# oxfordcontrol/Clarabel.rs

Measured on NVIDIA H100. Metric: ipm_iterations_per_sec, higher is better.
Workload: dtype f64

## Files before the change

clarabel.rs_b200/csrc/ldl.cu:

```cuda
#include <cuda_runtime.h>
#include <dlfcn.h>

#include <cmath>
#include <cstdio>
#include <cstring>
#include <algorithm>
#include <thread>
#include <vector>

#include "../../include/clarabel_b200.h"
#include "ldl_device.h"
#include "symbolic.h"
#include "vec.cuh"

namespace cb {

std::atomic<unsigned long long> g_launches{0};

typedef struct ncclComm* cb_ncclComm_t;
typedef struct { char internal[128]; } cb_ncclUniqueId;
struct NcclApi {
  void* lib = nullptr;
  int (*GetUniqueId)(cb_ncclUniqueId*) = nullptr;
  int (*CommInitRank)(cb_ncclComm_t*, int, cb_ncclUniqueId, int) = nullptr;
  int (*AllGather)(const void*, void*, size_t, int, cb_ncclComm_t, cudaStream_t) = nullptr;
  int (*CommDestroy)(cb_ncclComm_t) = nullptr;
  const char* (*GetErrorString)(int) = nullptr;
};
static NcclApi* nccl_api(const char* libpath) {
  static NcclApi api;
  static bool tried = false;
  if (api.lib) return &api;
  if (tried && !libpath) return nullptr;
  tried = true;
  void* h = dlopen(libpath && *libpath ? libpath : "libnccl.so.2", RTLD_NOW | RTLD_GLOBAL);
  if (!h) { std::fprintf(stderr, "[clarabel_b200] dlopen(%s) failed: %s\n", libpath ? libpath : "libnccl.so.2", dlerror()); return nullptr; }
  api.GetUniqueId = (int (*)(cb_ncclUniqueId*))dlsym(h, "ncclGetUniqueId");
  api.CommInitRank = (int (*)(cb_ncclComm_t*, int, cb_ncclUniqueId, int))dlsym(h, "ncclCommInitRank");
  api.AllGather = (int (*)(const void*, void*, size_t, int, cb_ncclComm_t, cudaStream_t))dlsym(h, "ncclAllGather");
  api.CommDestroy = (int (*)(cb_ncclComm_t))dlsym(h, "ncclCommDestroy");
  api.GetErrorString = (const char* (*)(int))dlsym(h, "ncclGetErrorString");
  if (!api.GetUniqueId || !api.CommInitRank || !api.AllGather || !api.CommDestroy) return nullptr;
  api.lib = h;
  return &api;
}



template <int NT>
__device__ __forceinline__ void pivot_inverse(double* A, int lda, int ns) {
  for (int j = threadIdx.x; j < ns; j += NT) {
    for (int i = j + 1; i < ns; i++) {
      double a0 = A[(long long)j * lda + i], a1 = 0.0;
      int k = j + 1;
      for (; k + 1 < i; k += 2) {
        a0 += A[(long long)k * lda + i] * A[(long long)k * lda + j];
        a1 += A[(long long)(k + 1) * lda + i] * A[(long long)(k + 1) * lda + j];
      }
      if (k < i) a0 += A[(long long)k * lda + i] * A[(long long)k * lda + j];
      A[(long long)i * lda + j] = -(a0 + a1);
    }
  }
}
template <int NT>
__device__ __forceinline__ void pivot_inverse_place(double* A, int lda, int ns) {
  for (int idx = threadIdx.x; idx < ns * ns; idx += NT) {
    const int j = idx / ns, i = idx - j * ns;
    if (i > j) {
      A[(long long)j * lda + i] = A[(long long)i * lda + j];
      A[(long long)i * lda + j] = 0.0;
    }
  }
}

template <int NT>
__global__ void __launch_bounds__(NT) k_factor_level(LDLDev d, int task_base, int smem_cap) {
  extern __shared__ double sm[];
  __shared__ double sD[CB_MAX_PANEL];
  __shared__ double sInv[CB_MAX_PANEL];
  const int tid = threadIdx.x;
  const int lane = tid & 31, warp = tid >> 5, nwarp = NT >> 5;
  const int s = d.level_tasks[task_base + blockIdx.x];
  const int f = d.sn_first[s];
  const int ns = d.sn_first[s + 1] - f;
  const long long rp = d.sn_rowptr[s];
  const int nr = (int)(d.sn_rowptr[s + 1] - rp);
  const int ld = ns + nr;
  double* __restrict__ P = d.L + d.panel_off[s];
  double* __restrict__ U = d.U + d.upd_off[s];
  const long long psz = (long long)ld * ns;
  const bool use_sm = psz <= (long long)smem_cap;
  double* W = use_sm ? sm : P;

  for (long long i = tid; i < psz; i += NT) W[i] = 0.0;
  __syncthreads();
  for (long long e = d.asm_ptr[s] + tid; e < d.asm_ptr[s + 1]; e += NT)
    W[d.asm_dst[e]] = d.vals[d.asm_src[e]];

  int c_reg = 0, c_pos = 0, c_zero = 0, c_nonf = 0;
  for (int j = 0; j < ns; j++) {
    __syncthreads();
    const double* __restrict__ cj = W + (long long)j * ld;
    double dj = cj[j];
    bool reg = false;
    if (d.reg_enable) {
      const double sg = (double)d.dsigns[f + j];
      if (dj * sg < d.reg_eps) { dj = d.reg_delta * sg; reg = true; }
    }
    const double inv = 1.0 / dj;
    if (tid == 0) {
      c_reg += reg ? 1 : 0;
      c_pos += dj > 0.0 ? 1 : 0;
      if (dj == 0.0) c_zero = 1;
      if (!isfinite(inv)) c_nonf = 1;
      d.D[f + j] = dj;
      d.Dinv[f + j] = inv;
      sD[j] = dj;
      sInv[j] = inv;
    }
    for (int k = j + 1 + warp; k < ns; k += nwarp) {
      const double wk = cj[k] * inv;
      double* __restrict__ ck = W + (long long)k * ld;
      for (int i = k + lane; i < ld; i += 32) ck[i] -= cj[i] * wk;
    }
  }
  __syncthreads();
  for (int j = warp; j < ns; j += nwarp) {
    double* __restrict__ cj = W + (long long)j * ld;
    const double inv = sInv[j];
    if (lane == 0) cj[j] = sD[j];
    for (int i = j + 1 + lane; i < ld; i += 32) cj[i] *= inv;
  }
  if (tid == 0) {
    if (c_reg) atomicAdd(&d.status[ST_REGCOUNT], c_reg);
    if (c_pos) atomicAdd(&d.status[ST_POSINERTIA], c_pos);
    if (c_zero) atomicExch(&d.status[ST_ZEROPIV], 1);
    if (c_nonf) atomicExch(&d.status[ST_NONFINITE], 1);
  }
  __syncthreads();

  {
    int it = 0;
    for (int b0 = 0; b0 < nr; b0 += 4)
      for (int a0 = b0; a0 < nr; a0 += 32, it++) {
        if (it % nwarp != warp) continue;
        const int a = a0 + lane;
        const bool on = a < nr;
        const int nb = min(4, nr - b0);
        double acc[4] = {0.0, 0.0, 0.0, 0.0};
        const double* __restrict__ ck = W + ns;
        for (int k = 0; k < ns; k++, ck += ld) {
          const double la = on ? ck[a] : 0.0, dk = sD[k];
#pragma unroll
          for (int c = 0; c < 4; c++) acc[c] += la * (ck[b0 + min(c, nb - 1)] * dk);
        }
#pragma unroll
        for (int c = 0; c < 4; c++)
          if (on && b0 + c < nr && a >= b0 + c) U[(long long)(b0 + c) * nr + a] = 0.0 - acc[c];
      }
  }
  if (ns > CB_SOLVE_SMALL_NS) {
    pivot_inverse<NT>(W, ld, ns);
    __syncthreads();
    pivot_inverse_place<NT>(W, ld, ns);
  }
  if (use_sm) {
    __syncthreads();
    for (long long i = tid; i < psz; i += NT) P[i] = W[i];
  }
}

#define LEAF1_NT 256
#define LEAF1_MAXLD 128
static_assert(LEAF1_MAXLD > CB_BIG_NR, "a level-0 column must fit the per-warp buffer");
__global__ void __launch_bounds__(LEAF1_NT) k_factor_leaf1(LDLDev d, int task_base, int count) {
  __shared__ double s_col[LEAF1_NT / 32][LEAF1_MAXLD];
  __shared__ int s_pos, s_reg;
  const int lane = threadIdx.x & 31, warp = threadIdx.x >> 5;
  const int i = blockIdx.x * (LEAF1_NT / 32) + warp;
  if (threadIdx.x == 0) { s_pos = 0; s_reg = 0; }
  __syncthreads();
  if (i < count) {
    double* col = s_col[warp];
    const int s = d.level_tasks[task_base + i];
    const int f = d.sn_first[s];
    const long long rp = d.sn_rowptr[s];
    const int nr = (int)(d.sn_rowptr[s + 1] - rp);
    const int ld = 1 + nr;
    double* __restrict__ P = d.L + d.panel_off[s];
    double* __restrict__ U = d.U + d.upd_off[s];
    for (int a = lane; a < ld; a += 32) col[a] = 0.0;
    __syncwarp();
    for (long long e = d.asm_ptr[s] + lane; e < d.asm_ptr[s + 1]; e += 32) col[d.asm_dst[e]] = d.vals[d.asm_src[e]];
    __syncwarp();
    double dj = col[0];
    bool reg = false;
    if (d.reg_enable) {
      const double sg = (double)d.dsigns[f];
      if (dj * sg < d.reg_eps) { dj = d.reg_delta * sg; reg = true; }
    }
    const double inv = 1.0 / dj;
    if (lane == 0) {
      if (dj == 0.0) atomicExch(&d.status[ST_ZEROPIV], 1);
      if (!isfinite(inv)) atomicExch(&d.status[ST_NONFINITE], 1);
      if (dj > 0.0) atomicAdd(&s_pos, 1);
      if (reg) atomicAdd(&s_reg, 1);
      d.D[f] = dj;
      d.Dinv[f] = inv;
    }
    __syncwarp();
    for (int a = lane; a < ld; a += 32) {
      const double v = a == 0 ? dj : col[a] * inv;
      col[a] = v;
      P[a] = v;
    }
    __syncwarp();
    for (int idx = lane; idx < nr * nr; idx += 32) {
      const int b = idx / nr, a = idx - b * nr;
      if (a >= b) {
        const double t = col[1 + b] * dj;
        double acc = 0.0;
        acc += col[1 + a] * t;
        U[idx] = 0.0 - acc;
      }
    }
  }
  __syncthreads();
  if (threadIdx.x == 0) {
    if (s_pos) atomicAdd(&d.status[ST_POSINERTIA], s_pos);
    if (s_reg) atomicAdd(&d.status[ST_REGCOUNT], s_reg);
  }
}

__global__ void k_permute_in(int n, const int* __restrict__ perm, const double* __restrict__ b,
                             double* __restrict__ xp) {
  int k = blockIdx.x * blockDim.x + threadIdx.x;
  if (k < n) xp[k] = b[perm[k]];
}

__device__ __forceinline__ unsigned long long df_gtime() {
#ifdef CB_EMU
  return 0;
#else
  unsigned long long t;
  asm volatile("mov.u64 %0, %%globaltimer;" : "=l"(t));
  return t;
#endif
}
__device__ __forceinline__ void df_wait_zero(volatile int* p) {
  unsigned ns = 20;
  while (*p > 0) { __nanosleep(ns); if (ns < 640) ns <<= 1; }
}
__device__ __forceinline__ void df_wait_set(volatile int* p) {
  unsigned ns = 20;
  while (*p == 0) { __nanosleep(ns); if (ns < 640) ns <<= 1; }
}

#include "ldl_solve.cuh"

#define DF_NT 256
#define DF_SMEM_DOUBLES (CB_PB_MAXNS * CB_PB_LD + 2 * CB_PB_MAXNS + CB_PB_MAXNS * 128)

__device__ __forceinline__ double ldcg_d(const double* p) { return __ldcg(p); }

template <class Map>
__device__ __forceinline__ void df_apply_sorted(double* base, const double* __restrict__ U,
                                                const int* __restrict__ esrc, const int* __restrict__ edst,
                                                int e0, int e1, Map map) {
  const int cnt = e1 - e0;
  if (cnt <= 0) return;
  const int per = (cnt + DF_NT - 1) / DF_NT;
  int b = e0 + threadIdx.x * per, e = min(e1, b + per);
  if (b >= e1) return;
  if (b > e0) { while (b < e1 && edst[b] == edst[b - 1]) b++; }
  if (e < e1) { while (e < e1 && edst[e] == edst[e - 1]) e++; }
  int i = b;
  while (i < e) {
    const int dd = edst[i];
    double acc = 0.0;
    while (i < e && edst[i] == dd) { acc += __ldcg(U + esrc[i]); i++; }
    const long long t = map(dd);
    if (t >= 0) base[t] += acc;
  }
}

__shared__ int df_cur_qi;
#define DF_STAMP(q, slot) do { if ((q).trace && threadIdx.x == 0) (q).trace[10 * (size_t)df_cur_qi + (slot)] = df_gtime(); } while (0)
__device__ __forceinline__ void df_front_complete(const DFFactor& q, int s) {
  const int p = q.parent[s];
  if (p >= 0) atomicSub(q.pend + p, 1);
}

__device__ void dff_small(const LDLDev& d, int s, double* sm, int* s_flag) {
  __shared__ double s_inv;
  const int tid = threadIdx.x, lane = tid & 31, warp = tid >> 5, nwarp = DF_NT >> 5;
  const int f = d.sn_first[s];
  const int ns = d.sn_first[s + 1] - f;
  const long long rp = d.sn_rowptr[s];
  const int nr = (int)(d.sn_rowptr[s + 1] - rp);
  const int ld = ns + nr;
  double* P = d.L + d.panel_off[s];
  double* U = d.U + d.upd_off[s];
  const long long psz = (long long)ld * ns;
  double* sD = sm;
  double* Wsm = sm + CB_MAX_PANEL;
  const bool use_sm = psz <= (long long)(DF_SMEM_DOUBLES - CB_MAX_PANEL);
  double* W = use_sm ? Wsm : P;
  (void)s_flag;
  for (long long i = tid; i < psz; i += DF_NT) W[i] = 0.0;
  for (int b = warp; b < nr; b += nwarp)
    for (int a = b + lane; a < nr; a += 32) U[(long long)b * nr + a] = 0.0;
  __syncthreads();
  for (long long e = d.asm_ptr[s] + tid; e < d.asm_ptr[s + 1]; e += DF_NT) W[d.asm_dst[e]] = d.vals[d.asm_src[e]];
  __syncthreads();
  for (long long ci = d.child_ptr[s]; ci < d.child_ptr[s + 1]; ci++) {
    const int c = d.child_list[ci];
    const long long crp = d.sn_rowptr[c];
    const int nrc = (int)(d.sn_rowptr[c + 1] - crp);
    const double* Uc = d.U + d.upd_off[c];
    const int* __restrict__ relc = d.rel + crp;
    for (int b = warp; b < nrc; b += nwarp) {
      const int rb = relc[b];
      for (int a = b + lane; a < nrc; a += 32) {
        const int ra = relc[a];
        const double v = __ldcg(Uc + (long long)b * nrc + a);
        if (rb < ns) W[(long long)rb * ld + ra] += v;
        else U[(long long)(rb - ns) * nr + (ra - ns)] += v;
      }
    }
    __syncthreads();
  }
  int c_reg = 0, c_pos = 0, c_zero = 0, c_nonf = 0;
  for (int j = 0; j < ns; j++) {
    if (tid == 0) {
      double dj = W[(long long)j * ld + j];
      if (d.reg_enable) {
        const double sg = (double)d.dsigns[f + j];
        if (dj * sg < d.reg_eps) { dj = d.reg_delta * sg; c_reg++; }
      }
      if (dj == 0.0) c_zero = 1;
      if (dj > 0.0) c_pos++;
      const double inv = 1.0 / dj;
      if (!isfinite(inv)) c_nonf = 1;
      d.D[f + j] = dj;
      d.Dinv[f + j] = inv;
      W[(long long)j * ld + j] = dj;
      s_inv = inv;
      sD[j] = dj;
    }
    __syncthreads();
    const double inv = s_inv;
    const double* cj = W + (long long)j * ld;
    for (int k = j + 1 + warp; k < ns; k += nwarp) {
      const double wk = cj[k] * inv;
      double* ck = W + (long long)k * ld;
      for (int i = k + lane; i < ld; i += 32) ck[i] -= cj[i] * wk;
    }
    __syncthreads();
    double* cjw = W + (long long)j * ld;
    for (int i = j + 1 + tid; i < ld; i += DF_NT) cjw[i] *= inv;
  }
  __syncthreads();
  if (tid == 0) {
    if (c_reg) atomicAdd(&d.status[ST_REGCOUNT], c_reg);
    if (c_pos) atomicAdd(&d.status[ST_POSINERTIA], c_pos);
    if (c_zero) atomicExch(&d.status[ST_ZEROPIV], 1);
    if (c_nonf) atomicExch(&d.status[ST_NONFINITE], 1);
  }
  for (int b = warp; b < nr; b += nwarp)
    for (int a = b + lane; a < nr; a += 32) {
      double acc = 0.0;
      for (int k = 0; k < ns; k++) {
        const double* ck = W + (long long)k * ld + ns;
        acc += ck[a] * (ck[b] * sD[k]);
      }
      U[(long long)b * nr + a] -= acc;
    }
  if (ns > CB_SOLVE_SMALL_NS) {
    pivot_inverse<DF_NT>(W, ld, ns);
    __syncthreads();
    pivot_inverse_place<DF_NT>(W, ld, ns);
    __syncthreads();
  }
  if (use_sm) for (long long i = tid; i < psz; i += DF_NT) P[i] = W[i];
}

#define DF_DCAP 32
#define DF_REC_INTS ((int)(sizeof(DFChildRec) / sizeof(int)))
#define DF_REC_INT(r, field) (reinterpret_cast<const int*>(r)[offsetof(DFChildRec, field) / sizeof(int)])

template <int NH>
__device__ __forceinline__ void df_add_child(const LDLDev& d, const DFChildRec& ch, double* dst, int rowoff,
                                             int rstride, int coloff, int cstride) {
  const int lane = threadIdx.x & 31, warp = threadIdx.x >> 5;
  const int* __restrict__ relc = d.rel + ch.relp;
  const double* Uc = d.U + ch.uoff;
  __syncwarp();
  if (ch.contig == 3) {
    const int r0 = ch.ra0 - rowoff - ch.a0, c0 = ch.rb0 - coloff - ch.b0;
    const int bfirst = ch.b0 + ((warp - (c0 + ch.b0)) & 7);
    const int a1 = ch.a1, b1 = ch.b1;
    for (int ab = ch.a0; ab < a1; ab += 32 * NH) {
      double v[8][NH];
#pragma unroll
      for (int c = 0; c < 8; c++) {
        const int b = bfirst + 8 * c;
#pragma unroll
        for (int h = 0; h < NH; h++) {
          const int a = ab + lane + 32 * h;
          v[c][h] = (b < b1 && a < a1 && a >= b) ? __ldcg(Uc + (long long)b * ch.nrc + a) : 0.0;
        }
      }
#pragma unroll
      for (int c = 0; c < 8; c++) {
        const int b = bfirst + 8 * c;
#pragma unroll
        for (int h = 0; h < NH; h++) {
          const int a = ab + lane + 32 * h;
          if (b < b1 && a < a1 && a >= b) dst[(r0 + a) * rstride + (c0 + b) * cstride] += v[c][h];
        }
      }
    }
    __syncwarp();
    return;
  }
  const int bl = ch.b0 + lane, bh = bl + 32;
  const int dc0 = bl < ch.b1 ? relc[bl] - coloff : -1;
  const int dc1 = bh < ch.b1 ? relc[bh] - coloff : -1;
  unsigned m0 = __ballot_sync(0xffffffffu, dc0 >= 0 && (dc0 & 7) == warp);
  unsigned m1 = __ballot_sync(0xffffffffu, dc1 >= 0 && (dc1 & 7) == warp);
  const int cnt0 = __popc(m0), cnt = cnt0 + __popc(m1);
  const int oc = lane >> 2, ar = lane & 3;
  int pos = -1;
  if (oc < cnt) {
    unsigned m = oc < cnt0 ? m0 : m1;
    const int skip = oc < cnt0 ? oc : oc - cnt0;
    for (int k = 0; k < skip; k++) m &= m - 1;
    pos = __ffs(m) - 1 + (oc < cnt0 ? 0 : 32);
  }
  const int srcl = pos < 0 ? 0 : (pos & 31);
  const int x0 = __shfl_sync(0xffffffffu, dc0, srcl), x1 = __shfl_sync(0xffffffffu, dc1, srcl);
  if (pos >= 0) {
    const int dcc = (pos < 32 ? x0 : x1) * cstride;
    const int b = ch.b0 + pos;
    const double* ucol = Uc + (long long)b * ch.nrc;
    const int a1 = ch.a1;
    for (int a = max(ch.a0, b) + ar; a < a1; a += 32) {
      double v[8];
      int r[8];
#pragma unroll
      for (int u = 0; u < 8; u++) {
        const int aa = a + 4 * u;
        const bool ok = aa < a1;
        v[u] = ok ? __ldcg(ucol + aa) : 0.0;
        r[u] = ok ? relc[aa] : rowoff;
      }
#pragma unroll
      for (int u = 0; u < 8; u++)
        if (a + 4 * u < a1) dst[(r[u] - rowoff) * rstride + dcc] += v[u];
    }
  }
  __syncwarp();
}

#define DF_ENT_FAST (2 * DF_NT)
struct DFEnt { int dd[2]; double v[2]; };
__device__ __forceinline__ void df_ent_issue(const double* __restrict__ U, const int* __restrict__ esrc,
                                             const int* __restrict__ edst, int e0, int e1, DFEnt& pe) {
  const int cnt = e1 - e0;
  pe.dd[0] = pe.dd[1] = -1;
  pe.v[0] = pe.v[1] = 0.0;
  if (cnt > DF_ENT_FAST) return;
  int src[2] = {0, 0};
#pragma unroll
  for (int u = 0; u < 2; u++) {
    const int i = threadIdx.x + u * DF_NT;
    if (i < cnt) { pe.dd[u] = edst[e0 + i]; src[u] = esrc[e0 + i]; }
  }
#pragma unroll
  for (int u = 0; u < 2; u++)
    if (threadIdx.x + u * DF_NT < cnt) pe.v[u] = __ldcg(U + src[u]);
}
template <class Map>
__device__ __forceinline__ void df_ent_apply(double* base, const double* __restrict__ U, const int* __restrict__ esrc,
                                             const int* __restrict__ edst, int e0, int e1, const DFEnt& pe,
                                             int* s_ed, double* s_ev, Map map) {
  const int cnt = e1 - e0;
  if (cnt <= 0) return;
  if (cnt > DF_ENT_FAST) { df_apply_sorted(base, U, esrc, edst, e0, e1, map); return; }
#pragma unroll
  for (int u = 0; u < 2; u++) {
    const int i = threadIdx.x + u * DF_NT;
    if (i < cnt) { s_ed[i] = pe.dd[u]; s_ev[i] = pe.v[u]; }
  }
  __syncthreads();
#pragma unroll
  for (int u = 0; u < 2; u++) {
    int i = threadIdx.x + u * DF_NT;
    if (i < cnt) {
      const int dd = pe.dd[u];
      if (i == 0 || s_ed[i - 1] != dd) {
        double acc = 0.0;
        while (i < cnt && s_ed[i] == dd) { acc += s_ev[i]; i++; }
        const long long t = map(dd);
        if (t >= 0) base[t] += acc;
      }
    }
  }
}

template <class Put>
__device__ __forceinline__ void df_scatter_asm(const LDLDev& d, int s, Put put) {
  const long long e0 = d.asm_ptr[s], e1 = d.asm_ptr[s + 1];
  for (long long e = e0 + threadIdx.x; e < e1; e += 4 * DF_NT) {
    long long dst[4];
    int src[4];
    double v[4];
#pragma unroll
    for (int u = 0; u < 4; u++) {
      const long long ee = e + (long long)u * DF_NT;
      const bool ok = ee < e1;
      dst[u] = ok ? (long long)d.asm_dst[ee] : -1;
      src[u] = ok ? d.asm_src[ee] : 0;
    }
#pragma unroll
    for (int u = 0; u < 4; u++) v[u] = dst[u] >= 0 ? d.vals[src[u]] : 0.0;
#pragma unroll
    for (int u = 0; u < 4; u++) if (dst[u] >= 0) put(dst[u], v[u]);
  }
}

template <class F>
__device__ __forceinline__ void df_children(const DFFactor& q, int d0, int d1, int* s_desc, F f) {
  for (int base = d0; base < d1; base += DF_DCAP) {
    const int cnt = min(DF_DCAP, d1 - base);
    const int* src = reinterpret_cast<const int*>(q.recs);
    for (int i = threadIdx.x; i < cnt * DF_REC_INTS; i += DF_NT) s_desc[i] = src[(size_t)base * DF_REC_INTS + i];
    __syncthreads();
    const DFChildRec* rec = reinterpret_cast<const DFChildRec*>(s_desc);
    for (int k = 0; k < cnt; k++) f(rec[k]);
    __syncthreads();
  }
}

__device__ void dff_diag(const LDLDev& d, const DFFactor& q, const DFTask& tk, double* sm, int* s_desc, int* s_ed, double* s_ev) {
  double* sA = sm;
  double* sSign = sm + CB_PB_MAXNS * CB_PB_LD;
  double* colbuf = sSign + CB_PB_MAXNS;
  const int tid = threadIdx.x;
  const int s = tk.s, ns = tk.ns, nr = tk.nr, f = tk.f;
  const int ld = ns + nr;
  const long long poff = tk.poff;
  double* P = d.L + poff;
  DFEnt pe;
  df_ent_issue(d.U, d.sc_panel_src, d.sc_panel_dst, tk.e0, tk.e1, pe);
  for (int i = tid; i < CB_PB_MAXNS * CB_PB_LD; i += DF_NT) sA[i] = 0.0;
  if (tid < CB_PB_MAXNS) sSign[tid] = tid < ns ? (double)d.dsigns[f + tid] : 1.0;
  __syncthreads();
  df_scatter_asm(d, s, [&](long long dst, double v) {
    const int col = (int)(dst / ld), row = (int)(dst - (long long)col * ld);
    if (row < ns) sA[col * CB_PB_LD + row] = v;
  });
  __syncthreads();
  df_children(q, tk.d0, tk.d1, s_desc, [&](const DFChildRec& ch) { df_add_child<2>(d, ch, sA, 0, 1, 0, CB_PB_LD); });
  df_ent_apply(sA, d.U, d.sc_panel_src, d.sc_panel_dst, tk.e0, tk.e1, pe, s_ed, s_ev,
               [&](int dd) -> long long { const int col = dd / ld, row = dd - col * ld; return row < ns ? (long long)col * CB_PB_LD + row : -1; });
  __syncthreads();
  DF_STAMP(q, 4);
  const int bi = tid & 15, bj = tid >> 4;
  const bool active = bi >= bj;
  double a[4][4];
#pragma unroll
  for (int k = 0; k < 4; k++)
#pragma unroll
    for (int i = 0; i < 4; i++) a[i][k] = active ? sA[(4 * bj + k) * CB_PB_LD + 4 * bi + i] : 0.0;
  int c_reg = 0, c_pos = 0, c_zero = 0, c_nonf = 0;
  const int nJ = (ns + 3) >> 2;
  for (int J = 0; J < nJ; J++) {
#pragma unroll
    for (int jj = 0; jj < 4; jj++) {
      const int j = 4 * J + jj;
      if (j >= ns) break;
      double* buf = colbuf + (j & 1) * 72;
      if (bj == J && active) {
        if (bi == J) {
          double dj = a[jj][jj];
          if (d.reg_enable) {
            const double sg = sSign[j];
            if (dj * sg < d.reg_eps) { dj = d.reg_delta * sg; c_reg++; }
          }
          if (dj == 0.0) c_zero = 1;
          if (dj > 0.0) c_pos++;
          const double inv = __drcp_rn(dj);
          if (!isfinite(inv)) c_nonf = 1;
          a[jj][jj] = dj;
          buf[64] = dj;
          buf[65] = inv;
          d.D[f + j] = dj;
          d.Dinv[f + j] = inv;
        }
#pragma unroll
        for (int i = 0; i < 4; i++) buf[4 * bi + i] = a[i][jj];
      }
      __syncthreads();
      if (active && bj >= J) {
        const double inv = buf[65];
        double li[4];
#pragma unroll
        for (int i = 0; i < 4; i++) li[i] = buf[4 * bi + i];
        if (bj > J) {
#pragma unroll
          for (int k = 0; k < 4; k++) {
            const double wk = buf[4 * bj + k] * inv;
#pragma unroll
            for (int i = 0; i < 4; i++) a[i][k] -= li[i] * wk;
          }
        } else {
#pragma unroll
          for (int k = jj + 1; k < 4; k++) {
            const double wk = buf[4 * bj + k] * inv;
#pragma unroll
            for (int i = 0; i < 4; i++) a[i][k] -= li[i] * wk;
          }
#pragma unroll
          for (int i = 0; i < 4; i++)
            if (4 * bi + i > j) a[i][jj] *= inv;
        }
      }
    }
  }
  if (c_reg) atomicAdd(&d.status[ST_REGCOUNT], c_reg);
  if (c_pos) atomicAdd(&d.status[ST_POSINERTIA], c_pos);
  if (c_zero) atomicExch(&d.status[ST_ZEROPIV], 1);
  if (c_nonf) atomicExch(&d.status[ST_NONFINITE], 1);
#pragma unroll
  for (int k = 0; k < 4; k++) {
    const int col = 4 * bj + k;
    if (col < ns) {
#pragma unroll
      for (int i = 0; i < 4; i++) {
        const int row = 4 * bi + i;
        if (row < ns) P[(long long)col * ld + row] = row >= col ? a[i][k] : 0.0;
      }
    }
  }
}

__device__ void dff_rows(const LDLDev& d, const DFFactor& q, const DFTask& tk, double* sm, int* s_desc, int* s_ed, double* s_ev) {
  double* sA = sm;
  double* sDval = sm + CB_PB_MAXNS * CB_PB_LD;
  double* sDinv = sDval + CB_PB_MAXNS;
  double* sR = sDinv + CB_PB_MAXNS;
  const int tid = threadIdx.x;
  const int s = tk.s, blk = tk.a, ns = tk.ns, nr = tk.nr, f = tk.f;
  const int ld = ns + nr;
  double* P = d.L + tk.poff;
  const int r0 = blk * DF_RB, r1 = min(nr, r0 + DF_RB);
  const int g0 = ns + r0, g1 = ns + r1;
  DFEnt pe;
  df_ent_issue(d.U, d.sc_panel_src, d.sc_panel_dst, tk.e0, tk.e1, pe);
  for (int i = tid; i < CB_PB_MAXNS * DF_RB; i += DF_NT) sR[i] = 0.0;
  __syncthreads();
  df_scatter_asm(d, s, [&](long long dst, double v) {
    const int col = (int)(dst / ld), row = (int)(dst - (long long)col * ld);
    if (row >= g0 && row < g1) sR[col * DF_RB + row - g0] = v;
  });
  __syncthreads();
  df_children(q, tk.d0, tk.d1, s_desc, [&](const DFChildRec& ch) { df_add_child<4>(d, ch, sR, g0, 1, 0, DF_RB); });
  df_ent_apply(sR, d.U, d.sc_panel_src, d.sc_panel_dst, tk.e0, tk.e1, pe, s_ed, s_ev,
               [&](int dd) -> long long { const int col = dd / ld, row = dd - col * ld; return (row >= g0 && row < g1) ? (long long)col * DF_RB + row - g0 : -1; });
  __syncthreads();
  DF_STAMP(q, 4);
  if (tid == 0) { df_wait_set(q.diag_done + s); __threadfence(); }
  __syncthreads();
  DF_STAMP(q, 5);
  for (int idx = tid; idx < ns * ns; idx += DF_NT) {
    const int j = idx / ns, i = idx - j * ns;
    sA[j * CB_PB_LD + i] = __ldcg(P + (long long)j * ld + i);
  }
  if (tid < ns) { sDval[tid] = __ldcg(d.D + f + tid); sDinv[tid] = __ldcg(d.Dinv + f + tid); }
  __syncthreads();
  constexpr int JB = 16;
  const int r = tid;
  if (r < r1 - r0) {
    double* prow = sR + r;
    for (int jb = 0; jb < ns; jb += JB) {
      const int nj = min(JB, ns - jb);
      double t[JB];
#pragma unroll
      for (int jj = 0; jj < JB; jj++) t[jj] = jj < nj ? prow[(jb + jj) * DF_RB] : 0.0;
      for (int kb = 0; kb < jb; kb += JB) {
#pragma unroll
        for (int kk = 0; kk < JB; kk++) {
          const double wk = prow[(kb + kk) * DF_RB] * sDval[kb + kk];
          const double2* lk2 = reinterpret_cast<const double2*>(sA + (kb + kk) * CB_PB_LD + jb);
#pragma unroll
          for (int j2 = 0; j2 < JB / 2; j2++) { const double2 l = lk2[j2]; t[2 * j2] -= wk * l.x; t[2 * j2 + 1] -= wk * l.y; }
        }
      }
#pragma unroll
      for (int jj = 0; jj < JB; jj++) {
        if (jj < nj) {
          const double* lk = sA + (jb + jj) * CB_PB_LD + jb;
#pragma unroll
          for (int j2 = jj + 1; j2 < JB; j2++) t[j2] -= t[jj] * lk[j2];
        }
      }
#pragma unroll
      for (int jj = 0; jj < JB; jj++) if (jj < nj) prow[(jb + jj) * DF_RB] = t[jj] * sDinv[jb + jj];
    }
  }
  __syncthreads();
  const int nrow = r1 - r0;
  for (int idx = tid; idx < ns * DF_RB; idx += DF_NT) {
    const int j = idx / DF_RB, rr = idx - j * DF_RB;
    if (rr < nrow) P[(long long)j * ld + g0 + rr] = sR[idx];
  }
}

__device__ void dff_rows_invert(const LDLDev& d, const DFTask& tk, double* sm) {
  double* sA = sm;
  const int ns = tk.ns, ld = ns + tk.nr;
  double* P = d.L + tk.poff;
  pivot_inverse<DF_NT>(sA, CB_PB_LD, ns);
  __syncthreads();
  for (int idx = threadIdx.x; idx < ns * ns; idx += DF_NT) {
    const int j = idx / ns, i = idx - j * ns;
    if (i > j) P[(long long)j * ld + i] = sA[i * CB_PB_LD + j];
  }
}

__device__ void dff_tile(const LDLDev& d, const DFFactor& q, const DFTask& tk, double* sm, int* s_desc, int* s_ed, double* s_ev) {
  double* sAt = sm;
  double* sBt = sm + TS * TS;
  double* sC = sm + 2 * TS * TS;
  double* sD = sC + TS * (TS + 1);
  const int tid = threadIdx.x;
  const int ti = tk.a, tj = tk.b, ns = tk.ns, nr = tk.nr, f = tk.f;
  const int ld = ns + nr;
  const double* P = d.L + tk.poff;
  double* U = d.U + tk.uoff;
  const int i0 = ti * TS, j0 = tj * TS;
  const int ni = min(TS, nr - i0), nj = min(TS, nr - j0);
  DFEnt pe;
  df_ent_issue(d.U, d.sc_tile_src, d.sc_tile_dst, tk.e0, tk.e1, pe);
  {
    const int rr = tid & (TS - 1), kq = tid >> 6;
    const unsigned sa = (unsigned)__cvta_generic_to_shared(sAt), sb = (unsigned)__cvta_generic_to_shared(sBt);
    const unsigned za = rr < ni ? 8u : 0u, zb = rr < nj ? 8u : 0u;
    const double* pa = P + ns + i0 + (rr < ni ? rr : 0);
    const double* pb = P + ns + j0 + (rr < nj ? rr : 0);
#pragma unroll 4
    for (int k = kq; k < ns; k += 4) {
      const long long col = (long long)k * ld;
#ifdef CB_EMU
      (void)sa; (void)sb;
      sAt[k * TS + rr] = za ? pa[col] : 0.0;
      sBt[k * TS + rr] = zb ? pb[col] : 0.0;
    }
#else
      asm volatile("cp.async.ca.shared.global [%0], [%1], 8, %2;" ::"r"(sa + (unsigned)(k * TS + rr) * 8u), "l"(pa + col), "r"(za) : "memory");
      asm volatile("cp.async.ca.shared.global [%0], [%1], 8, %2;" ::"r"(sb + (unsigned)(k * TS + rr) * 8u), "l"(pb + col), "r"(zb) : "memory");
    }
    asm volatile("cp.async.commit_group;" ::: "memory");
#endif
    if (tid < ns) sD[tid] = __ldcg(d.D + f + tid);
  }
  DF_STAMP(q, 6);
#ifdef CB_EMU
  const int tx = tid & 15, ty = tid >> 4;
#define OWN_R(i) (tx + 16 * (i))
#define OWN_C(j) (ty + 16 * (j))
#else
  const int lk = tid & 3, lr = (tid & 31) >> 2, r0w = ((tid >> 5) & 1) * 32, c0w = (tid >> 6) * 16;
#define OWN_R(i) (r0w + 8 * (i) + lr)
#define OWN_C(j) (c0w + 8 * ((j) >> 1) + 2 * lk + ((j) & 1))
#endif
  double creg[4][4];
#pragma unroll
  for (int i = 0; i < 4; i++)
#pragma unroll
    for (int j = 0; j < 4; j++) creg[i][j] = 0.0;
  const int ndense = tk.ndense;
  for (int kd = 0; kd < ndense; kd++) {
    const DFChildRec* rec = q.recs + (size_t)(tk.d0 + kd);
    const long long uoff = rec->uoff;
    const int nrc = DF_REC_INT(rec, nrc), a0 = DF_REC_INT(rec, a0), a1 = DF_REC_INT(rec, a1), b0 = DF_REC_INT(rec, b0), b1 = DF_REC_INT(rec, b1);
    const int ra = a0 - (DF_REC_INT(rec, ra0) - (ns + i0)), rb = b0 - (DF_REC_INT(rec, rb0) - (ns + j0));
    const double* Uc = d.U + uoff;
    double v[4][4];
#pragma unroll
    for (int j = 0; j < 4; j++) {
      const int b = OWN_C(j) + rb;
#pragma unroll
      for (int i = 0; i < 4; i++) {
        const int a = OWN_R(i) + ra;
        v[i][j] = (a >= a0 && a < a1 && b >= b0 && b < b1 && a >= b) ? __ldcg(Uc + (long long)b * nrc + a) : 0.0;
      }
    }
#pragma unroll
    for (int i = 0; i < 4; i++)
#pragma unroll
      for (int j = 0; j < 4; j++) creg[i][j] += v[i][j];
  }
  const bool use_sc = (tk.d1 - tk.d0 > ndense) || (tk.e1 > tk.e0);
  if (use_sc) {
    for (int idx = tid; idx < TS * (TS + 1); idx += DF_NT) sC[idx] = 0.0;
    __syncthreads();
    DF_STAMP(q, 7);
    df_children(q, tk.d0 + ndense, tk.d1, s_desc, [&](const DFChildRec& ch) { df_add_child<2>(d, ch, sC, ns + i0, TS + 1, ns + j0, 1); });
    DF_STAMP(q, 8);
    df_ent_apply(sC, d.U, d.sc_tile_src, d.sc_tile_dst, tk.e0, tk.e1, pe, s_ed, s_ev, [&](int dd) -> long long { return dd; });
  }
#ifndef CB_EMU
  asm volatile("cp.async.wait_group 0;" ::: "memory");
#endif
  __syncthreads();
  for (int idx = tid; idx < ns * TS; idx += DF_NT) sBt[idx] *= sD[idx >> 6];
#ifndef CB_EMU
  {
    const int ns4 = (ns + 3) & ~3;
    for (int idx = ns * TS + tid; idx < ns4 * TS; idx += DF_NT) { sAt[idx] = 0.0; sBt[idx] = 0.0; }
  }
#endif
  __syncthreads();
  DF_STAMP(q, 4);
#ifdef CB_EMU
  double acc[4][4];
#pragma unroll
  for (int i = 0; i < 4; i++)
#pragma unroll
    for (int j = 0; j < 4; j++) acc[i][j] = 0.0;
#pragma unroll 4
  for (int k = 0; k < ns; k++) {
    double a[4], b[4];
#pragma unroll
    for (int i = 0; i < 4; i++) { a[i] = sAt[k * TS + tx + 16 * i]; b[i] = sBt[k * TS + ty + 16 * i]; }
#pragma unroll
    for (int i = 0; i < 4; i++)
#pragma unroll
      for (int j = 0; j < 4; j++) acc[i][j] += a[i] * b[j];
  }
#else
  double c2[4][2][2];
  {
#pragma unroll
    for (int i = 0; i < 4; i++)
#pragma unroll
      for (int j = 0; j < 2; j++) { c2[i][j][0] = 0.0; c2[i][j][1] = 0.0; }
    const int ns4 = (ns + 3) & ~3;
#pragma unroll 2
    for (int k = 0; k < ns4; k += 4) {
      double a[4], b[2];
#pragma unroll
      for (int i = 0; i < 4; i++) a[i] = sAt[(k + lk) * TS + r0w + 8 * i + lr];
#pragma unroll
      for (int j = 0; j < 2; j++) b[j] = sBt[(k + lk) * TS + c0w + 8 * j + lr];
#pragma unroll
      for (int i = 0; i < 4; i++)
#pragma unroll
        for (int j = 0; j < 2; j++)
          asm volatile("mma.sync.aligned.m8n8k4.row.col.f64.f64.f64.f64 {%0,%1}, {%2}, {%3}, {%0,%1};"
                       : "+d"(c2[i][j][0]), "+d"(c2[i][j][1]) : "d"(a[i]), "d"(b[j]));
    }
  }
#endif
  DF_STAMP(q, 5);
#pragma unroll
  for (int i = 0; i < 4; i++) {
    const int rr = OWN_R(i);
#pragma unroll
    for (int j = 0; j < 4; j++) {
      const int cc = OWN_C(j);
#ifdef CB_EMU
      const double prod = acc[i][j];
#else
      const double prod = c2[i][j >> 1][j & 1];
#endif
      if (rr < ni && cc < nj && (i0 + rr >= j0 + cc))
        U[(long long)(j0 + cc) * nr + (i0 + rr)] = (use_sc ? creg[i][j] + sC[rr * (TS + 1) + cc] : creg[i][j]) - prod;
    }
  }
#undef OWN_R
#undef OWN_C
}

__global__ void __launch_bounds__(DF_NT, 2) k_factor_df(LDLDev d, DFFactor q) {
  extern __shared__ __align__(16) double dfsm[];
  __shared__ __align__(16) int s_desc[DF_DCAP * DF_REC_INTS];
  __shared__ __align__(16) int s_task[16];
  __shared__ int s_ed[DF_ENT_FAST];
  __shared__ double s_ev[DF_ENT_FAST];
  __shared__ int s_last;
  const int tid = threadIdx.x;
  if (tid == 0) df_cur_qi = -1;
  for (;;) {
    __syncthreads();
    if (tid == 0) {
      if (q.trace && df_cur_qi >= 0) q.trace[10 * (size_t)df_cur_qi + 2] = df_gtime();
      const int qi = atomicAdd(q.qhead, 1);
      df_cur_qi = qi < q.ntask ? qi : -1;
      if (q.trace && df_cur_qi >= 0) {
        unsigned smid = 0;
#ifndef CB_EMU
        asm volatile("mov.u32 %0, %%smid;" : "=r"(smid));
#endif
        q.trace[10 * (size_t)qi] = df_gtime();
        q.trace[10 * (size_t)qi + 3] = smid;
      }
    }
    __syncthreads();
    const int qi = df_cur_qi;
    if (qi < 0) break;
    if (tid < 4) reinterpret_cast<int4*>(s_task)[tid] = q.tasks[4 * (size_t)qi + tid];
    __syncthreads();
    const DFTask& tk = *reinterpret_cast<const DFTask*>(s_task);
    const int kind = tk.kind, s = tk.s;
    if (kind == 0) {
      if (tid == 0) { df_wait_zero(q.pend + s); __threadfence(); if (q.trace) q.trace[10 * (size_t)qi + 1] = df_gtime(); }
      __syncthreads();
      dff_small(d, s, dfsm, nullptr);
      __syncthreads();
      if (tid == 0) { __threadfence(); df_front_complete(q, s); }
    } else if (kind == 1) {
      if (tid == 0) { df_wait_zero(q.pend + s); __threadfence(); if (q.trace) q.trace[10 * (size_t)qi + 1] = df_gtime(); }
      __syncthreads();
      dff_diag(d, q, tk, dfsm, s_desc, s_ed, s_ev);
      __syncthreads();
      if (tid == 0) { __threadfence(); atomicExch(q.diag_done + s, 1); }
    } else if (kind == 2) {
      if (tid == 0) { df_wait_zero(q.pend + s); __threadfence(); if (q.trace) q.trace[10 * (size_t)qi + 1] = df_gtime(); }
      __syncthreads();
      dff_rows(d, q, tk, dfsm, s_desc, s_ed, s_ev);
      __syncthreads();
      if (tid == 0) { __threadfence(); s_last = atomicSub(q.rows_left + s, 1) == 1; }
      __syncthreads();
      if (s_last && tk.ns > CB_SOLVE_SMALL_NS) dff_rows_invert(d, tk, dfsm);
    } else {
      if (tid == 0) { df_wait_zero(q.rows_left + s); __threadfence(); if (q.trace) q.trace[10 * (size_t)qi + 1] = df_gtime(); }
      __syncthreads();
      dff_tile(d, q, tk, dfsm, s_desc, s_ed, s_ev);
      __syncthreads();
      if (tid == 0) {
        __threadfence();
        if (atomicSub(q.tiles_left + s, 1) == 1) df_front_complete(q, s);
      }
    }
  }
}

#include "ldl_selinv.cuh"
#include "ldl_schur.cuh"

__global__ void k_update_values(double* __restrict__ vals, const int* __restrict__ idx,
                                const double* __restrict__ v, long long len) {
  long long i = (long long)blockIdx.x * blockDim.x + threadIdx.x;
  if (i < len) vals[idx[i]] = v[i];
}
__global__ void k_scale_values(double* __restrict__ vals, const int* __restrict__ idx, double s,
                               long long len) {
  long long i = (long long)blockIdx.x * blockDim.x + threadIdx.x;
  if (i < len) vals[idx[i]] *= s;
}
__global__ void k_offset_values(double* __restrict__ vals, const int* __restrict__ idx, double off,
                                const signed char* __restrict__ sg, long long len) {
  long long i = (long long)blockIdx.x * blockDim.x + threadIdx.x;
  if (i < len) {
    const int s = sg[i];
    if (s > 0) vals[idx[i]] += off;
    else if (s < 0) vals[idx[i]] -= off;
  }
}


#define CK(x)                                                                        \
  do {                                                                               \
    cudaError_t e_ = (x);                                                            \
    if (e_ != cudaSuccess) {                                                         \
      std::fprintf(stderr, "[clarabel_b200] CUDA error %s at %s:%d\n",              \
                   cudaGetErrorString(e_), __FILE__, __LINE__);                      \
      return CLDL_E_CUDA;                                                            \
    }                                                                                \
  } while (0)

int LDLObject::init(int n_, const int64_t* Ap, const int32_t* Ai, const double* Ax,
                    const int8_t* dsigns, const cldl_opts& o, const int* perm_in) {
  n = n_;
  opts = o;
  int ndev = 0;
  if (cudaGetDeviceCount(&ndev) != cudaSuccess || ndev == 0) {
    std::fprintf(stderr, "[clarabel_b200] no CUDA device: this backend has no CPU fallback\n");
    return CLDL_E_CUDA;
  }
  device = o.device;
  CK(cudaSetDevice(device));
  SymbolicOptions so;
  so.ordering = o.ordering ? o.ordering : ORDER_BEST;
  so.amd_dense_scale = o.amd_dense_scale > 0 ? o.amd_dense_scale : 1.5;
  if (o.max_panel > 0) so.max_panel = o.max_panel > CB_PB_MAXNS ? CB_PB_MAXNS : o.max_panel;
  if (o.nd_leaf > 0) so.nd_leaf = o.nd_leaf;
  cb_tmark(nullptr);
  schur = !schur_set.empty();
  int rc = schur ? analyse_schur(n, Ap, Ai, perm_in, schur_set, so, S) : analyse(n, Ap, Ai, perm_in, so, S);
  cb_tmark("ldl: ordering + symbolic");
  if (rc == -2) return CLDL_E_EMPTY_COLUMN;
  if (rc == -3) return CLDL_E_NOT_TRIU;
  if (rc == -5) return CLDL_E_BAD_PERM;
  if (rc) return CLDL_E_ARG;
  shard_nranks = o.shard_nranks > 1 ? o.shard_nranks : 1;
  shard_rank = o.shard_rank;
  if (schur && sharded()) return CLDL_E_ARG;
  if (schur) shard_rank = 0;
  if (sharded()) {
    if (shard_rank < 0 || shard_rank >= shard_nranks) return CLDL_E_ARG;
    std::vector<int> par(S.sn_parent);
    if (plan_shards(S.nsup, S.sn_first.data(), S.sn_rowptr.data(), par.data(), shard_nranks, shard)) return CLDL_E_ARG;
    shard_cut.assign(shard_nranks, {});
    shard_xidx.assign(shard_nranks, {});
    for (int s = 0; s < S.nsup; s++) {
      const int g = shard.owner[s];
      if (g < 0) continue;
      if (S.sn_parent[s] >= 0 && shard.owner[S.sn_parent[s]] < 0) shard_cut[g].push_back(s);
      for (int j = S.sn_first[s]; j < S.sn_first[s + 1]; j++) shard_xidx[g].push_back(S.perm[j]);
    }
  }
  const std::vector<int> owner = schur ? schur_owner(S, n - (int)schur_set.size()) : shard.owner;

  CK(cudaStreamCreateWithFlags(&stream, cudaStreamNonBlocking));
  CK(cudaStreamCreateWithFlags(&stream_a, cudaStreamNonBlocking));
  CK(cudaStreamCreateWithFlags(&stream_b, cudaStreamNonBlocking));
  for (auto& e : ev_leaf) CK(cudaEventCreateWithFlags(&e, cudaEventDisableTiming));
  CK(cudaEventCreate(&ev0));
  CK(cudaEventCreate(&ev1));
  CK(cudaMallocHost((void**)&h_status, ST_COUNT * sizeof(int)));

  auto to_ll = [](const std::vector<int64_t>& v) { return std::vector<long long>(v.begin(), v.end()); };
  CK(upload(&dev.sn_first, S.sn_first));
  CK(upload(&dev.sn_rowptr, to_ll(S.sn_rowptr)));
  CK(upload(&dev.sn_rows, S.sn_rows));
  CK(upload(&dev.child_ptr, to_ll(S.child_ptr)));
  CK(upload(&dev.child_list, S.child_list));
  CK(upload(&dev.rel, S.rel));
  CK(upload(&dev.panel_off, to_ll(S.panel_off)));
  CK(upload(&dev.upd_off, to_ll(S.upd_off)));
  CK(upload(&dev.asm_ptr, to_ll(S.asm_ptr)));
  CK(upload(&dev.asm_src, S.asm_src));
  CK(upload(&dev.asm_dst, to_ll(S.asm_dst)));
  CK(upload(&dev.perm, S.perm));
  {
    std::vector<signed char> ds(n);
    for (int k = 0; k < n; k++) ds[k] = dsigns ? (signed char)dsigns[S.perm[k]] : (signed char)1;
    CK(upload(&dev.dsigns, ds));
  }
  nnzA = Ap[n];
  h_colptr.assign(Ap, Ap + n + 1);
  h_rowval.assign(Ai, Ai + nnzA);
  CK(cudaMalloc((void**)&dev.vals, (size_t)(nnzA ? nnzA : 1) * sizeof(double)));
  CK(cudaMemcpy(dev.vals, Ax, (size_t)nnzA * sizeof(double), cudaMemcpyHostToDevice));
  big_alloc_rc = 0;
  big_alloc = std::thread([this]() {
    if (cudaSetDevice(device) != cudaSuccess) { big_alloc_rc = 1; return; }
    const size_t nu = S.sn_rows.size() ? S.sn_rows.size() : 1;
    if (cudaMalloc((void**)&dev.L, ((size_t)(S.L_alloc ? S.L_alloc : 1) + 8) * sizeof(double)) != cudaSuccess ||
        cudaMalloc((void**)&dev.U, (size_t)(S.upd_total ? S.upd_total : 1) * sizeof(double)) != cudaSuccess ||
        cudaMalloc((void**)&dev.u, nu * sizeof(double)) != cudaSuccess ||
        cudaMalloc((void**)&d_u2, nu * sizeof(double)) != cudaSuccess)
      big_alloc_rc = 1;
  });
  struct BigJoin { std::thread& t; ~BigJoin() { if (t.joinable()) t.join(); } } big_join{big_alloc};
  CK(cudaMalloc((void**)&dev.D, (size_t)n * sizeof(double)));
  CK(cudaMalloc((void**)&dev.Dinv, (size_t)n * sizeof(double)));
  CK(cudaMalloc((void**)&d_xp, (size_t)n * sizeof(double)));
  CK(cudaMalloc((void**)&d_xp2, (size_t)n * sizeof(double)));
  CK(cudaMalloc((void**)&d_bx, (size_t)2 * n * sizeof(double)));
  CK(cudaMalloc((void**)&dev.status, ST_COUNT * sizeof(int)));
  CK(cudaMemset(dev.status, 0, ST_COUNT * sizeof(int)));
  dev.reg_enable = o.regularize_enable;
  dev.reg_eps = o.regularize_eps;
  dev.reg_delta = o.regularize_delta;

  cb_tmark("ldl: uploads + device alloc");
  int max_optin = 0, nsm = 0;
  CK(cudaDeviceGetAttribute(&max_optin, cudaDevAttrMaxSharedMemoryPerBlockOptin, device));
  CK(cudaDeviceGetAttribute(&nsm, cudaDevAttrMultiProcessorCount, device));
  const int level_cap = (max_optin - 2048) / 8;
  const size_t extra2 = (size_t)2 * (2 * CB_PB_MAXNS + SV_MAXROWS + 4 * CB_PB_MAXNS) * sizeof(double);
  {
    const size_t per_cta = ((size_t)227 * 1024) / SV_MINB - 1024 - 64;
    sv_cap = (int)((per_cta - extra2) / sizeof(double)) - 2;
    sv_cap &= ~1;
    sv_cap = std::min(sv_cap, 16384);
  }
  SolvePlan sp;
  std::thread th_solve([&]() { sp = build_solve_plan(S, owner, shard_rank, sv_cap); });
  struct ThJoin { std::thread& t; ~ThJoin() { if (t.joinable()) t.join(); } } th_solve_guard{th_solve};
  Level0Plan l0 = build_level0_plan(S, owner, shard_rank, level_cap);
  FactorPlan fp = build_factor_plan(S, owner, shard_rank);
  th_solve.join();
  cb_tmark("ldl: plans");

  CK(cudaFuncSetAttribute(k_factor_level<256>, cudaFuncAttributeMaxDynamicSharedMemorySize, level_cap * 8));
  plan = std::move(l0.segs);
  CK(upload(&dev.level_tasks, l0.level_tasks));

  CK(upload(&dev.sc_panel_src, fp.sc_panel_src));
  CK(upload(&dev.sc_panel_dst, fp.sc_panel_dst));
  CK(upload(&dev.sc_tile_src, fp.sc_tile_src));
  CK(upload(&dev.sc_tile_dst, fp.sc_tile_dst));
  if (std::getenv("CB_TIMING")) std::fprintf(stderr, "[cb timing]     factor plan: %zu tasks, %zu child records, %zu big fronts, %zu tiles\n",
                                              fp.tasks.size(), fp.recs.size(), fp.sc_panel_ptr.size() - 1, fp.sc_tile_ptr.size() - 1);
  dff.ntask = (int)fp.tasks.size();
  dff_ntask_owned = fp.ntask_owned;
  CK(upload(&dff.tasks, fp.tasks));
  CK(upload(&dff.recs, fp.recs));
  CK(upload(&d_dff_init, fp.cnt_init));
  CK(cudaMalloc((void**)&d_dff_cnt, fp.cnt_init.size() * sizeof(int) + 16));
  dff.pend = d_dff_cnt; dff.diag_done = d_dff_cnt + S.nsup; dff.rows_left = d_dff_cnt + 2 * (size_t)S.nsup;
  dff.tiles_left = d_dff_cnt + 3 * (size_t)S.nsup;
  CK(cudaMalloc((void**)&dff.qhead, sizeof(int)));
  CK(upload(&dff.parent, S.sn_parent));
  CK(upload(&dff.big_pos, fp.big_pos));
  CK(upload(&dff.tile_base, fp.tile_base));
  CK(cudaFuncSetAttribute(k_factor_df, cudaFuncAttributeMaxDynamicSharedMemorySize, DF_SMEM_DOUBLES * 8));
  int occ = 0;
  CK(cudaOccupancyMaxActiveBlocksPerMultiprocessor(&occ, k_factor_df, DF_NT, (size_t)DF_SMEM_DOUBLES * 8));
  dff_grid = nsm * std::max(1, occ);
  dff_nsup4 = 4 * (size_t)S.nsup;
  if (std::getenv("CB_DF_TRACE") && dff.ntask > 0) {
    h_dff_tasks = fp.tasks;
    CK(cudaMalloc((void**)&dff.trace, (size_t)dff.ntask * 10 * sizeof(unsigned long long)));
    CK(cudaMemset(dff.trace, 0, (size_t)dff.ntask * 10 * sizeof(unsigned long long)));
  }

  const int nt = (int)sp.tasks.size();
  sv_nwide = (int)sp.wide.size();
  sv_nleaf1 = (int)sp.leaf1.size(); sv_nleafn = (int)sp.leafn.size(); sv_nleafw = (int)sp.leafw.size();
  sv_leafw_nrmax = sp.leafw_nrmax;
  sv_leafw_grid = sv_nleafw;
  sv_ntask_owned = sp.ntask_owned;
  CK(upload(&dev.gat_ptr, sp.gat_ptr));
  CK(upload(&dev.gat_src, sp.gat_src));
  CK(upload(&d_sv_leaf1, sp.leaf1));
  CK(upload(&d_sv_leafn, sp.leafn));
  CK(upload(&d_sv_leafw, sp.leafw));
  CK(upload(&sv.fronts, sp.fronts));
  CK(upload(&sv.front2task, sp.front2task));
  CK(upload(&sv.parent, S.sn_parent));
  CK(upload(&sv.tasks, sp.tasks));
  sv_ninit = sp.cnt_init.size();
  sv_nzero = (size_t)nt + 2 * (size_t)S.nsup + 2;
  CK(upload(&d_sv_init, sp.cnt_init));
  CK(cudaMalloc((void**)&d_sv_cnt, (sv_ninit + sv_nzero) * sizeof(int)));
  sv.pend = d_sv_cnt; sv.fleft = d_sv_cnt + nt; sv.bleft = sv.fleft + S.nsup;
  sv.tdone = d_sv_cnt + sv_ninit; sv.ydone = sv.tdone + nt; sv.done = sv.ydone + S.nsup; sv.qhead = sv.done + S.nsup;
  sv.bpart_stride = (long long)(sp.nslots ? sp.nslots : 1) * CB_PB_MAXNS;
  CK(cudaMalloc((void**)&sv.bpart, (size_t)2 * sv.bpart_stride * sizeof(double)));
  sv.ntask = nt;
  for (int nr2 = 1; nr2 <= 2; nr2++)
    sv_smem[nr2 - 1] = ((size_t)sv_cap + 2 + (size_t)nr2 * (2 * CB_PB_MAXNS + SV_MAXROWS + 4 * CB_PB_MAXNS)) * sizeof(double);
  if ((rc = sv_configure())) return rc;
  const int sv_occ = sv_occupancy();
  if (sv_occ < 1) return CLDL_E_CUDA;
  sv_grid = nsm * sv_occ;
  use_dataflow = true;
  if (std::getenv("CB_DF_TRACE_SOLVE") && nt > 0) {
    CK(cudaMalloc((void**)&sv.trace, (size_t)nt * 8 * sizeof(unsigned long long)));
    CK(cudaMemset(sv.trace, 0, (size_t)nt * 8 * sizeof(unsigned long long)));
    h_sv_tasks = sp.tasks;
  }
  if (std::getenv("CB_TIMING") != nullptr) std::fprintf(stderr, "[cb timing]     solve plan: %d tasks (%d leaf columns, %d narrow leaves, %d wide leaves, %d wide fronts, %d row slabs), slab %d doubles, %d CTAs\n",
                                   nt, sv_nleaf1, sv_nleafn, sv_nleafw, sv_nwide, sp.nslots, sv_cap, sv_grid);
  cb_tmark("ldl: plan uploads");
  if (sharded()) {
    d_shard_xidx.assign(shard_nranks, nullptr);
    for (int w = 0; w < 2; w++) { d_shard_segs[w].assign(shard_nranks, nullptr); shard_nsegs[w].assign(shard_nranks, 0); }
    for (int g = 0; g < shard_nranks; g++) CK(upload(&d_shard_xidx[g], shard_xidx[g]));
  }
  if (schur && (rc = schur_setup(sp))) return rc;
  if (big_alloc.joinable()) big_alloc.join();
  if (big_alloc_rc) { std::fprintf(stderr, "[clarabel_b200] device allocation of the factor storage failed\n"); return CLDL_E_CUDA; }
  cb_tmark("ldl: big allocations joined");
  CK(cudaDeviceSynchronize());
  factored = false;
  return CLDL_OK;
}

void LDLObject::release() {
  cudaSetDevice(device);
  for (auto& w : d_shard_segs) for (auto& p : w) if (p) { cudaFree(p); p = nullptr; }
  for (int* p : d_shard_xidx) if (p) cudaFree(p);
  d_shard_xidx.clear();
  if (nccl_comm) { if (NcclApi* a = nccl_api(nullptr)) a->CommDestroy((cb_ncclComm_t)nccl_comm); nccl_comm = nullptr; }
  if (d_xsend) { cudaFree(d_xsend); d_xsend = nullptr; }
  if (d_xrecv) { cudaFree(d_xrecv); d_xrecv = nullptr; }
  xbuf_cap = 0;
  auto fr = [](const void* p) { if (p) cudaFree((void*)p); };
  fr(dev.sn_first); fr(dev.sn_rowptr); fr(dev.sn_rows); fr(dev.child_ptr); fr(dev.child_list);
  fr(dev.rel); fr(dev.panel_off); fr(dev.upd_off); fr(dev.asm_ptr); fr(dev.asm_src);
// ... 931 lines not shown
```

Before: 26.25.

## Compact diagonal LDL block to triangular warps with shrinking named barriers

The dense diagonal-block LDL factorization now maps only the lower-triangular 4x4 tiles onto the first five warps, using a packed triangular index. The remaining warps zero the upper panel and exit. Block-wide __syncthreads is replaced by a named barrier whose participant count shrinks as finished leading warps drop out. The next pivot column is published early inside the current step, which shortens the critical path and removes idle threads from each barrier. In exchange the barrier-count logic is subtle, and an emulation fallback barrier is added.

Result: no change. 26.41 (median of 6 runs) (+0.6%).

```diff
diff --git a/clarabel.rs_b200/csrc/ldl.cu b/clarabel.rs_b200/csrc/ldl.cu
--- a/clarabel.rs_b200/csrc/ldl.cu
+++ b/clarabel.rs_b200/csrc/ldl.cu
@@ -285,6 +285,18 @@
 }
 
 __shared__ int df_cur_qi;
+#ifdef CB_EMU
+__shared__ int df_bar_arrived;
+__shared__ int df_bar_gen;
+__device__ __forceinline__ void df_bar_sync(int n) {
+  volatile int* gen = &df_bar_gen;
+  const int g = *gen;
+  if (atomicAdd(&df_bar_arrived, 1) == n - 1) { df_bar_arrived = 0; *gen = g + 1; }
+  else while (*gen == g) __nanosleep(20);
+}
+#else
+__device__ __forceinline__ void df_bar_sync(int n) { __barrier_sync_count(1, n); }
+#endif
 #define DF_STAMP(q, slot) do { if ((q).trace && threadIdx.x == 0) (q).trace[10 * (size_t)df_cur_qi + (slot)] = df_gtime(); } while (0)
 __device__ __forceinline__ void df_front_complete(const DFFactor& q, int s) {
   const int p = q.parent[s];
@@ -543,6 +555,8 @@
   }
 }
 
+#define DF_DW 5
+#define DF_TRI0(b) (16 * (b) - (b) * ((b) - 1) / 2)
 __device__ void dff_diag(const LDLDev& d, const DFFactor& q, const DFTask& tk, double* sm, int* s_desc, int* s_ed, double* s_ev) {
   double* sA = sm;
   double* sSign = sm + CB_PB_MAXNS * CB_PB_LD;
@@ -567,68 +581,91 @@
                [&](int dd) -> long long { const int col = dd / ld, row = dd - col * ld; return row < ns ? (long long)col * CB_PB_LD + row : -1; });
   __syncthreads();
   DF_STAMP(q, 4);
-  const int bi = tid & 15, bj = tid >> 4;
-  const bool active = bi >= bj;
+  const int warp = tid >> 5;
+  if (warp >= DF_DW) {
+    for (int idx = tid - 32 * DF_DW; idx < CB_PB_MAXNS * CB_PB_MAXNS; idx += DF_NT - 32 * DF_DW) {
+      const int col = idx >> 6, row = idx & 63;
+      if (col < ns && (row >> 2) < (col >> 2)) P[(long long)col * ld + row] = 0.0;
+    }
+    return;
+  }
+  int bi = 0, bj = 0;
+  const bool active = tid < DF_TRI0(16);
+  if (active) {
+    while (tid >= DF_TRI0(bj + 1)) bj++;
+    bi = bj + tid - DF_TRI0(bj);
+  }
   double a[4][4];
 #pragma unroll
   for (int k = 0; k < 4; k++)
 #pragma unroll
     for (int i = 0; i < 4; i++) a[i][k] = active ? sA[(4 * bj + k) * CB_PB_LD + 4 * bi + i] : 0.0;
   int c_reg = 0, c_pos = 0, c_zero = 0, c_nonf = 0;
+  auto publish = [&](const int kk, const int jn) {
+    double* nb = colbuf + (jn & 1) * 72;
+    if (bi == bj) {
+      double dj = a[kk][kk];
+      if (d.reg_enable) {
+        const double sg = sSign[jn];
+        if (dj * sg < d.reg_eps) { dj = d.reg_delta * sg; c_reg++; }
+      }
+      if (dj == 0.0) c_zero = 1;
+      if (dj > 0.0) c_pos++;
+      const double inv = __drcp_rn(dj);
+      if (!isfinite(inv)) c_nonf = 1;
+      a[kk][kk] = dj;
+      nb[64] = dj;
+      nb[65] = inv;
+      d.D[f + jn] = dj;
+      d.Dinv[f + jn] = inv;
+    }
+#pragma unroll
+    for (int i = 0; i < 4; i++) nb[4 * bi + i] = a[i][kk];
+  };
+  if (active && bj == 0) publish(0, 0);
   const int nJ = (ns + 3) >> 2;
   for (int J = 0; J < nJ; J++) {
+    const int w0 = DF_TRI0(J) >> 5, wp = DF_TRI0(J ? J - 1 : 0) >> 5;
 #pragma unroll
     for (int jj = 0; jj < 4; jj++) {
       const int j = 4 * J + jj;
       if (j >= ns) break;
-      double* buf = colbuf + (j & 1) * 72;
-      if (bj == J && active) {
-        if (bi == J) {
-          double dj = a[jj][jj];
-          if (d.reg_enable) {
-            const double sg = sSign[j];
-            if (dj * sg < d.reg_eps) { dj = d.reg_delta * sg; c_reg++; }
-          }
-          if (dj == 0.0) c_zero = 1;
-          if (dj > 0.0) c_pos++;
-          const double inv = __drcp_rn(dj);
-          if (!isfinite(inv)) c_nonf = 1;
-          a[jj][jj] = dj;
-          buf[64] = dj;
-          buf[65] = inv;
-          d.D[f + j] = dj;
-          d.Dinv[f + j] = inv;
-        }
-#pragma unroll
-        for (int i = 0; i < 4; i++) buf[4 * bi + i] = a[i][jj];
-      }
-      __syncthreads();
+      df_bar_sync(32 * (DF_DW - (jj == 0 ? wp : w0)));
+      if (warp < w0) break;
+      const double* buf = colbuf + (j & 1) * 72;
       if (active && bj >= J) {
         const double inv = buf[65];
         double li[4];
 #pragma unroll
         for (int i = 0; i < 4; i++) li[i] = buf[4 * bi + i];
+        auto upd = [&](const int k) {
+          const double wk = buf[4 * bj + k] * inv;
+#pragma unroll
+          for (int i = 0; i < 4; i++) a[i][k] -= li[i] * wk;
+        };
         if (bj > J) {
-#pragma unroll
-          for (int k = 0; k < 4; k++) {
-            const double wk = buf[4 * bj + k] * inv;
-#pragma unroll
-            for (int i = 0; i < 4; i++) a[i][k] -= li[i] * wk;
+          upd(0);
+          if (jj == 3 && bj == J + 1 && j + 1 < ns) publish(0, j + 1);
+          upd(1);
+          upd(2);
+          upd(3);
+        } else {
+          if (jj < 3) {
+            upd(jj + 1);
+            if (j + 1 < ns) publish(jj + 1, j + 1);
           }
-        } else {
-#pragma unroll
-          for (int k = jj + 1; k < 4; k++) {
-            const double wk = buf[4 * bj + k] * inv;
-#pragma unroll
-            for (int i = 0; i < 4; i++) a[i][k] -= li[i] * wk;
-          }
+#pragma unroll
+          for (int k = jj + 2; k < 4; k++) upd(k);
 #pragma unroll
           for (int i = 0; i < 4; i++)
             if (4 * bi + i > j) a[i][jj] *= inv;
         }
       }
     }
-  }
+    if (warp < w0) break;
+  }
+  if (q.trace && tid == DF_TRI0(16) - 1) q.trace[10 * (size_t)df_cur_qi + 5] = df_gtime();
+  if (!active) return;
   if (c_reg) atomicAdd(&d.status[ST_REGCOUNT], c_reg);
   if (c_pos) atomicAdd(&d.status[ST_POSINERTIA], c_pos);
   if (c_zero) atomicExch(&d.status[ST_ZEROPIV], 1);
@@ -894,6 +931,9 @@
   __shared__ int s_last;
   const int tid = threadIdx.x;
   if (tid == 0) df_cur_qi = -1;
+#ifdef CB_EMU
+  if (tid == 0) df_bar_arrived = 0;
+#endif
   for (;;) {
     __syncthreads();
     if (tid == 0) {
```
